# burritojustice/reporter

Hardware: AMD Instinct MI355X
Metric: GPS points matched/sec (whole node) at 1/2/4/8 MI355X; % segment-ID agreement vs meili (higher is better)
Workload: dtype f32

## Files before the change

reporter_amd/csrc/abi.cpp:

```cpp
#include <dlfcn.h>

#include <algorithm>
#include <atomic>
#include <chrono>
#include <cmath>
#include <condition_variable>
#include <cstdio>
#include <cstdlib>
#include <cstring>
#include <deque>
#include <fstream>
#include <exception>
#include <functional>
#include <memory>
#include <mutex>
#include <new>
#include <sstream>
#include <thread>

#include "engine.h"
#include "javastr.h"
#include "json.h"
#include "pyrepr.h"
#include "report.h"
// ... 1735 lines not shown
  E->nbins = dev_counts ? nbins : 0;
  E->bin_kph = bin_kph;
  return OTM_OK;
}

int otm_hist_bind(otm_engine* E, void* dev_counts, int nbins, float bin_kph) {
  return otm_hist_bind_ex(E, dev_counts, nbins, bin_kph, nullptr);
}

int otm_graph_info(const otm_engine* E, int64_t* n_nodes, int64_t* n_edges, int64_t* n_segments) {
  if (!E) return fail(OTM_EINVAL, "engine is NULL");
  if (!E->members.empty()) E = E->members[0];
  if (n_nodes) *n_nodes = E->host.h.n_nodes;
  if (n_edges) *n_edges = E->host.h.n_edges;
  if (n_segments) *n_segments = E->host.h.n_segments;
  return OTM_OK;
}

int otm_index_info(const otm_engine* E, float* rmax, int64_t* entries, int32_t* incomplete_rows, float* build_ms) {
  if (!E) return fail(OTM_EINVAL, "engine is NULL");
  if (!E->members.empty()) E = E->members[0];
  if (rmax) *rmax = E->idx.rmax;
  if (entries) *entries = E->index_entries;
  if (incomplete_rows) *incomplete_rows = E->index_incomplete_rows;
  if (build_ms) *build_ms = E->index_build_ms;
  return OTM_OK;
}

int otm_index_tables(const otm_engine* E, int64_t* slots, int64_t* bytes, int32_t* load_pct) {
  if (!E) return fail(OTM_EINVAL, "engine is NULL");
  if (!E->members.empty()) E = E->members[0];
  const int64_t n = E->index_slots + E->index_near_slots;
  if (slots) *slots = n;
  if (bytes) *bytes = n * otm::IDX_SLOT_BYTES;
  if (load_pct) *load_pct = E->idx.rmax > 0.0f ? E->idx.load_pct : 0;
  return OTM_OK;
}

int otm_index_levels(const otm_engine* E, float* radii, int64_t* entries, int cap) {
  if (!E) return fail(OTM_EINVAL, "engine is NULL");
  if (!E->members.empty()) E = E->members[0];
  int n = 0;
  for (int l = 0; l < otm::NEAR_LEVELS; ++l) {
    if (!(E->idxn[l].rmax > 0.0f)) continue;
    if (n < cap) {
      if (radii) radii[n] = E->idxn[l].rmax;
      if (entries) entries[n] = E->index_near_level_entries[l];
    }
    ++n;
  }
  return n;
}

int otm_grid_info(const otm_engine* E, double* cell_deg, int32_t* rows, int32_t* cols, int64_t* entries,
                  int32_t* mult) {
  if (!E) return fail(OTM_EINVAL, "engine is NULL");
  if (!E->members.empty()) E = E->members[0];
  if (cell_deg) *cell_deg = E->g.cell;
  if (rows) *rows = E->grid_rows;
  if (cols) *cols = E->grid_cols;
  if (entries) *entries = E->grid_entries;
  if (mult) *mult = E->grid_mult;
  return OTM_OK;
}

int otm_set_counting(otm_engine* E, int on) {
  if (!E) return fail(OTM_EINVAL, "engine is NULL");
// ... 173 lines not shown
```

reporter_amd/csrc/engine.cpp:

```cpp
#include "engine.h"

#include <algorithm>
#include <chrono>
#include <cmath>
#include <cstdlib>

#include <cstring>

namespace otm {

#define HIPCHK(x)                                                              \
  do {                                                                         \
    hipError_t e_ = (x);                                                       \
    if (e_ != hipSuccess) {                                                    \
      *err = std::string(#x) + ": " + hipGetErrorString(e_);                   \
      return OTM_EDEVICE;                                                      \
    }                                                                          \
  } while (0)

static int ensure(otm_engine::Buf& b, size_t bytes, std::string* err);
static int ensure_pinned(otm_engine::Buf& b, size_t bytes, std::string* err) {
  if (bytes == 0) bytes = 16;
  if (b.cap >= bytes) return OTM_OK;
  if (b.p) (void)hipHostFree(b.p);
// ... 297 lines not shown

int create_stream(int slot, hipStream_t* s, bool own_queue) {
  (void)slot;
  if (own_queue) {
    int dev = 0, ncu = 0;
    if (hipGetDevice(&dev) == hipSuccess &&
        hipDeviceGetAttribute(&ncu, hipDeviceAttributeMultiprocessorCount, dev) == hipSuccess && ncu > 0) {
      std::vector<uint32_t> mask((size_t)(ncu + 31) / 32, 0u);
      for (int c = 0; c < ncu; ++c) mask[(size_t)c / 32] |= 1u << (c % 32);
      if (hipExtStreamCreateWithCUMask(s, (uint32_t)mask.size(), mask.data()) == hipSuccess) return 0;
    }
  }
  return hipStreamCreateWithFlags(s, hipStreamNonBlocking) != hipSuccess;
}

int engine_clone(const otm_engine* P, otm_engine* C, std::string* err, bool own_queue) {
  C->parent = P;
  C->device = P->device;
  HIPCHK(hipSetDevice(C->device));
  const int slot = ++const_cast<otm_engine*>(P)->n_clones;
  if (create_stream(slot, &C->stream, own_queue)) {
    *err = "stream creation failed";
    return OTM_EDEVICE;
  }
  C->host.h = P->host.h;
  C->g = P->g;
  C->idx = P->idx;
  for (int l = 0; l < NEAR_LEVELS; ++l) C->idxn[l] = P->idxn[l];
  for (int l = 0; l < NEAR_LEVELS; ++l) C->index_near_level_entries[l] = P->index_near_level_entries[l];
  C->index_rmax = P->index_rmax;
  C->index_entries = P->index_entries;
  C->index_slots = P->index_slots;
  C->index_near_slots = P->index_near_slots;
  C->index_incomplete_rows = P->index_incomplete_rows;
  C->index_build_ms = P->index_build_ms;
  C->small_points = P->small_points;
  C->trans_lanes = P->trans_lanes;
  C->mc = P->mc;
  C->rc = P->rc;
  C->dp = P->dp;
  C->drc = P->drc;
  HIPCHK(hipMalloc((void**)&C->ctr, sizeof(DevCounters)));
  HIPCHK(hipMalloc((void**)&C->ctr_save, sizeof(DevCounters)));
  HIPCHK(hipMemset(C->ctr, 0, sizeof(DevCounters)));
  for (auto& e : C->kev) HIPCHK(hipEventCreate(&e));
  (void)err;
  return OTM_OK;
}

static float auto_index_radius(const otm_engine* E) {
  constexpr double INDEX_ROW_NODES = 140.0;
  const auto& h = E->host.h;
  const double lat_mid = 0.5 * (h.bbox[0] + h.bbox[2]) * 3.14159265358979323846 / 180.0;
  const double h_m = (h.bbox[2] - h.bbox[0]) * 111195.0;
  const double w_m = (h.bbox[3] - h.bbox[1]) * 111195.0 * std::cos(lat_mid);
  const double area = std::max(h_m * w_m, 1.0);
  const double rho = std::max((double)h.n_nodes, 1.0) / area;
  double r = std::sqrt(INDEX_ROW_NODES / (2.0 * rho));
  r = std::min(r, (double)E->dp.factor * (double)E->dp.breakage);
  return (float)(std::ceil(r / 50.0) * 50.0);
}

namespace {
struct IndexBuilt {
  DevIndex X{};
  int64_t entries = 0, slots = 0;
  int32_t incomplete = 0;
};
int build_index_at(otm_engine* E, float* r, bool shrink, size_t budget, IndexBuilt& out, std::string* err) {
  out = IndexBuilt{};
  const int32_t N = E->g.n_edges + E->g.n_nodes;
  hipStream_t s = E->stream;
  int32_t* row_cnt = nullptr;
  int64_t* row_off = nullptr;
  IdxRow* rows = nullptr;
  HIPCHK(hipMalloc(&row_cnt, ((size_t)N + 1) * 4));
  HIPCHK(hipMalloc(&row_off, ((size_t)N + 1) * 8));
  HIPCHK(hipMalloc(&rows, ((size_t)N + 1) * sizeof(IdxRow)));
  size_t tmpb = scan_tmp_bytes(N) + 256;
  void* tmp = nullptr;
  HIPCHK(hipMalloc(&tmp, tmpb));
  int64_t total = 0;
  int pct = index_load_fast();
  auto size_rows = [&](int load) -> int {
    launch_row_sizes(row_cnt, row_off, N, load, s);
    scan_i64(row_off, N, tmp, tmpb, s);
    launch_row_pack(row_cnt, row_off, rows, N, s);
    HIPCHK(hipMemcpyAsync(&total, row_off + N, 8, hipMemcpyDeviceToHost, s));
    HIPCHK(hipStreamSynchronize(s));
    return OTM_OK;
  };
  for (int attempt = 0;; ++attempt) {
    launch_index_build(E->g, E->dp.turn_units, index_cost_bound(*r), row_cnt, nullptr, nullptr, false, s);
    if (size_rows(pct)) return OTM_EDEVICE;
    if (pct != index_load_dense() && ((double)total + 1.0) * IDX_SLOT_BYTES > (double)budget) {
      pct = index_load_dense();
      if (size_rows(pct)) return OTM_EDEVICE;
    }
    const double need = ((double)total + 1.0) * IDX_SLOT_BYTES;
    if (need <= (double)budget) break;
    const float rr = (float)(std::floor(*r * std::sqrt((double)budget / need) * 0.9 / 50.0) * 50.0);
    if (!shrink || attempt == 4 || rr < 100.0f) {
      (void)hipFree(tmp);
      (void)hipFree(rows);
      (void)hipFree(row_off);
      (void)hipFree(row_cnt);
      *r = 0.0f;
      return OTM_OK;
    }
    *r = rr;
  }
  (void)hipFree(tmp);
  E->graph_allocs.push_back(row_cnt);
  E->graph_allocs.push_back(row_off);
  E->graph_allocs.push_back(rows);
  void* slot = nullptr;
  HIPCHK(hipMalloc(&slot, ((size_t)total + 1) * IDX_SLOT_BYTES));
  E->graph_allocs.push_back(slot);
  HIPCHK(hipMemsetAsync(slot, 0xFF, ((size_t)total + 1) * IDX_SLOT_BYTES, s));
  launch_index_build(E->g, E->dp.turn_units, index_cost_bound(*r), row_cnt, rows, (uint4*)slot, true, s);
  HIPCHK(hipGetLastError());
  std::vector<int32_t> cnt((size_t)N);
  HIPCHK(hipMemcpyAsync(cnt.data(), row_cnt, (size_t)N * 4, hipMemcpyDeviceToHost, s));
  HIPCHK(hipStreamSynchronize(s));
  for (int32_t c : cnt) {
    out.incomplete += c < 0;
    out.entries += c > 0 ? c : 0;
  }
  out.slots = total;
  out.X.rmax = *r;
  out.X.cmax = index_cost_bound(*r);
  out.X.row = rows;
  out.X.slot = (const uint4*)slot;
  out.X.load_pct = pct;
  return OTM_OK;
}

size_t index_budget() {
  if (const char* bm = std::getenv("OTM_INDEX_BUDGET_MB")) return (size_t)std::strtoull(bm, nullptr, 0) << 20;
  size_t fr = 0, tot = 0;
  if (hipMemGetInfo(&fr, &tot) != hipSuccess) return 0;
  return fr / 2;
}
}

int build_index(otm_engine* E, std::string* err) {
  E->idx = DevIndex{};
  for (auto& x : E->idxn) x = DevIndex{};
  E->idx.rmax = 0.0f;
  if (E->index_rmax < 0.0f) E->index_rmax = auto_index_radius(E);
  E->index_rmax = std::min(E->index_rmax, INDEX_RMAX_CAP);
  if (!(E->index_rmax > 0.0f)) return OTM_OK;
  hipStream_t s = E->stream;
  hipEvent_t a, z;
  HIPCHK(hipEventCreate(&a));
  HIPCHK(hipEventCreate(&z));
  HIPCHK(hipEventRecord(a, s));
  IndexBuilt full;
  int rc = build_index_at(E, &E->index_rmax, true, index_budget(), full, err);
  if (rc != OTM_OK) return rc;
  E->idx = full.X;
  E->index_entries = full.entries;
  E->index_slots = full.slots;
  E->index_incomplete_rows = full.incomplete;
  std::vector<float> radii;
  if (E->index_near_set) {
    radii = E->index_near_m;
  } else if ((double)full.slots * IDX_SLOT_BYTES >= OTM_INDEX_NEAR_MIN_GB * 1e9) {
    for (float f : std::initializer_list<float> OTM_INDEX_NEAR_FRACS) radii.push_back(E->index_rmax * f);
  }
  for (float& r : radii) r = (float)(std::floor(r / 50.0) * 50.0);
  std::sort(radii.begin(), radii.end());
  radii.erase(std::unique(radii.begin(), radii.end()), radii.end());
  int nl = 0;
  for (float rn : radii) {
    if (nl == NEAR_LEVELS || !(E->idx.rmax > 0.0f) || rn < 100.0f || rn >= E->idx.rmax) continue;
    IndexBuilt near;
    rc = build_index_at(E, &rn, false, index_budget(), near, err);
    if (rc != OTM_OK) return rc;
    if (rn > 0.0f) {
      E->index_near_level_entries[nl] = near.entries;
      E->index_near_slots += near.slots;
      E->idxn[nl++] = near.X;
    }
  }
  HIPCHK(hipEventRecord(z, s));
  HIPCHK(hipEventSynchronize(z));
  HIPCHK(hipEventElapsedTime(&E->index_build_ms, a, z));
  (void)hipEventDestroy(a);
  (void)hipEventDestroy(z);
  return OTM_OK;
}

void engine_free(otm_engine* E) {
  if (E->device >= 0) (void)hipSetDevice(E->device);
  for (void* p : E->graph_allocs) (void)hipFree(p);
  E->graph_allocs.clear();
  otm_engine::Buf* bufs[] = {
      &E->in_off,        &E->in_lat,       &E->in_lon,         &E->in_time,        &E->in_acc,     &E->in_blob,
      &E->pt_trace,
      &E->is_col,        &E->prevc,        &E->nextc,        &E->gc,             &E->ncand,          &E->cand_eo,      &E->cand_em,
      &E->cand_xeo,      &E->cand_xem,
      &E->probe,         &E->col_prev,     &E->kq_prev,        &E->vmeta,  &E->colrec, &E->colrec_pos,        &E->trans_off,      &E->trans,          &E->bp,         &E->state,      &E->chosen,
      &E->chain_start,   &E->route_dist,   &E->ipos,   &E->path_off,       &E->path_len,       &E->path_pool,  &E->trace_err,
      &E->overflow_list0, &E->overflow_list2, &E->counters_i32, &E->scan_tmp, &E->snap,   &E->big_key,
      &E->big_lab,       &E->big_inq,      &E->big_fr,         &E->big_ins,        &E->big_prev,
      &E->huge_key,      &E->huge_lab,     &E->huge_inq,       &E->huge_fr,        &E->huge_ins,         &E->huge_prev,
      &E->cbig_key,      &E->cbig_val,     &E->cbig_skey,
      &E->overflow_list3, &E->o_traces,       &E->o_seg_cnt,  &E->o_way_cnt,
      &E->o_segments,    &E->o_seg_gidx,   &E->o_way_ids,      &E->o_reports,  &E->o_rep_cnt,  &E->seg_ub,
      &E->f_seg_off,     &E->f_way_off,    &E->f_rep_off,      &E->f_segs,     &E->f_ways,     &E->f_reps,
      &E->f_traces,
      &E->abort_flag,    &E->rs_blob,      &E->ord_tile,      &E->ord_cnt,      &E->ord_cursor,     &E->ord_grp,    &E->ord_item,
      &E->d_req,         &E->req_cnt,      &E->req_ok,     &E->req_lat,    &E->req_lon,    &E->req_time,   &E->req_acc,
      &E->resp_hdr,      &E->resp_seg,     &E->resp_rep,       &E->resp_hlen,      &E->resp_slen,  &E->resp_rlen,
// ... 981 lines not shown
```

reporter_amd/csrc/engine.h:

```cpp
#pragma once
#include <atomic>
#include <hip/hip_runtime.h>

#include <condition_variable>
#include <deque>
#include <memory>
#include <mutex>
#include <string>
#include <thread>
#include <vector>

#include "kernels.h"
#include "otm_internal.h"
#include "otmatch.h"

struct ReqSlab {
  char* base = nullptr;
  size_t cap = 0;
  bool pinned = false;
};

namespace otm {
struct H2DOrder {
  std::mutex m;
// ... 5 lines not shown
};
}

struct otm_engine {
  const otm_engine* parent = nullptr;
  std::vector<otm_engine*> members;
  struct MemberPool* member_pool = nullptr;
  std::vector<otm_trace_result> g_traces;
  std::vector<otm_segment> g_segs;
  std::vector<otm_report_rec> g_reps;
  std::vector<int64_t> g_ways;
  int device = 0;
  std::atomic<int> n_clones{0};
  hipStream_t stream = nullptr;
  hipEvent_t sync_ev = nullptr;
  bool spin_waits = false;
  otm::HostGraph host;
  otm::DevGraph g{};
  std::vector<void*> graph_allocs;
  float index_rmax = -1.0f;
  int64_t small_points = 0;
  int trans_lanes = 8;
  int grid_mult = 0;
  int32_t grid_rows = 0, grid_cols = 0;
  int64_t grid_entries = 0;
  otm::DevIndex idx{};
  otm::DevIndex idxn[otm::NEAR_LEVELS]{};
  std::vector<float> index_near_m;
  bool index_near_set = false;
  int64_t index_near_level_entries[otm::NEAR_LEVELS]{};
  int64_t index_entries = 0;
  int64_t index_slots = 0;
  int64_t index_near_slots = 0;
  int32_t index_incomplete_rows = 0;
  float index_build_ms = 0.0f;
  otm::MatchConfig mc;
  otm::ReportConfig rc;
  otm::DevParams dp{};
  otm::DevReportCfg drc{};
  std::mutex mu;

  struct Buf {
    void* p = nullptr;
    size_t cap = 0;
  };
  Buf in_off, in_lat, in_lon, in_time, in_acc, in_blob;
  Buf pt_trace, is_col, prevc, nextc, gc, ncand, cand_eo, cand_em, cand_xeo, cand_xem, probe, col_prev, kq_prev, vmeta, colrec, colrec_pos, trans_off, trans, bp, state, chosen,
      chain_start, route_dist, ipos, path_off, path_len, path_pool, trace_err, overflow_list0, overflow_list2,
      counters_i32, scan_tmp, snap;
  Buf big_key, big_lab, big_inq, big_fr, big_ins, big_prev;
  Buf huge_key, huge_lab, huge_inq, huge_fr, huge_ins, huge_prev, overflow_list3;
  int32_t huge_log2 = 0;
  int32_t huge_ready_log2 = 0;
  Buf cbig_key, cbig_val, cbig_skey;
  int32_t cand_log2 = 0;
  int32_t huge_final = 0, cand_final = 0;
  int32_t last_attempts = 0;
  int32_t last_resumes = 0;
  Buf ord_tile, ord_cnt, ord_cursor, ord_grp, ord_item;
  Buf abort_flag;
  Buf rs_blob;
  int64_t trans_cap = 0;
  bool caps_read = false, caps_pinned = false;
  Buf o_traces, o_seg_cnt, o_way_cnt, o_rep_cnt, seg_ub, o_segments, o_seg_gidx, o_way_ids, o_reports;
  Buf f_seg_off, f_way_off, f_rep_off, f_segs, f_ways, f_reps, f_traces;
  otm::DevCounters* ctr = nullptr;
// ... 87 lines not shown
```

reporter_amd/csrc/kernels.h:

```cpp
#pragma once
#include <hip/hip_runtime.h>

#include <cstdint>

#include "otmatch.h"

namespace otm {

constexpr int KMAX = 32;
constexpr int KIN = 8;
static_assert(KIN == 4 || KIN == 8, "inline blocks of 4 or 8 slots (whole 16-B emission pieces)");
constexpr int KX = KMAX - KIN;
constexpr int MAX_HITS = 256;
constexpr int SEARCH_LIMIT = 98304;
constexpr int LDS_TABLE_CAP = 256;
constexpr int LDS_TABLE_LIMIT = 192;
constexpr int BIG_TABLE_LOG2 = 17;
constexpr int BIG_TABLE_CAP = 1 << BIG_TABLE_LOG2;
#ifndef OTM_BIG_SLOTS
#define OTM_BIG_SLOTS 512
#endif
constexpr int BIG_SLOTS = OTM_BIG_SLOTS;
constexpr int HUGE_SLOTS = 8;
constexpr int CAND_BIG_SLOTS = 64;
// ... 15 lines not shown
  const uint32_t* cell_off;
  const uint32_t* cell_ent;
  const float4* ent_geo;
  const uint16_t *e_head_out, *e_head_in;
  const uint32_t* e_len64;
  const uint4* e_rec;
  const int2* e_fl;
  const int64_t* way_tab;
  int32_t n_nodes, n_edges, n_segments, grid_rows, grid_cols;
  double lat0, lon0, cell;
  float bb_lat0, bb_lon0, bb_inv_h, bb_inv_w;
};

#ifndef OTM_ORDER_BITS
#define OTM_ORDER_BITS 6
#endif
constexpr int ORDER_BITS = OTM_ORDER_BITS;
constexpr int ORDER_SIDE = 1 << ORDER_BITS;
constexpr int ORDER_TILES = ORDER_SIDE * ORDER_SIDE;
constexpr int ORDER_GROUPS = 8;
struct DevOrder {
  int32_t* item;
  int32_t* grp;
  uint16_t* tile;
  int32_t* tile_cnt;
  int32_t* cursor;
};

struct IdxRow {
  int64_t off;
  int32_t cnt;
  uint32_t cap;
};
struct DevIndex {
  float rmax;
  uint32_t cmax;
  const IdxRow* row;
  const uint4* slot;
  int load_pct;
};
constexpr int IDX_SLOT_BYTES = 16;
constexpr float INDEX_RMAX_CAP = 200000.0f;
constexpr uint32_t NODE_KEY = 0x80000000u;
constexpr uint32_t NONE_PRED = 0xFFFFFFFFu;
constexpr int NEAR_LEVELS = 3;
#ifndef OTM_INDEX_NEAR_FRACS
#define OTM_INDEX_NEAR_FRACS {0.45f}
#endif
#ifndef OTM_INDEX_NEAR_MIN_GB
#define OTM_INDEX_NEAR_MIN_GB 16.0
#endif
constexpr int INDEX_BUILD_LOG2 = 11;
constexpr int INDEX_BUILD_CAP = 1 << INDEX_BUILD_LOG2;
constexpr int INDEX_BUILD_LIMIT = 1536;
__host__ __device__ inline uint32_t index_cost_bound(float B) { return (uint32_t)floor((double)B * 64.0); }

constexpr int ORDER_CAND = 1, ORDER_TRANS = 2, ORDER_ROUTE = 4;
constexpr int TURN_TABLE = 181;
constexpr uint32_t TURN_UNITS_MAX = 0xFFFFFFu;
constexpr uint32_t NO_TURNS = 0xFFFFFFFFu;
struct DevParams {
  float sigma_z, beta, factor, breakage, interp, search_radius, max_search_radius, gps_accuracy;
  const uint32_t* turn_units;
  int max_candidates;
  int order_mask;
  int cand_wave_all;
};

struct DevReportCfg {
  int n_report, n_transition;
// ... 138 lines not shown
void launch_transitions(const DevGraph& g, const DevBatch& b, const DevParams& p, DevWork& w, hipStream_t s,
                        const Marks& mk, int sub, int from = RESUME_ALL);
void launch_viterbi(const DevBatch& b, DevWork& w, hipStream_t s, const Marks& mk);
void launch_route(const DevGraph& g, const DevBatch& b, const DevParams& p, DevWork& w, hipStream_t s,
                  const Marks& mk, int from = RESUME_ALL);
void launch_segments(const DevGraph& g, const DevBatch& b, DevWork& w, DevOut& o, bool write, hipStream_t s,
                     const Marks& mk);
void launch_report(const DevBatch& b, const DevReportCfg& rc, DevWork& w, DevOut& o, hipStream_t s, const Marks& mk);
void launch_order(const DevBatch& b, DevWork& w, hipStream_t s, const Marks& mk);
void launch_seg_bound(const DevGraph& g, const DevBatch& b, const DevParams& p, DevWork& w, int64_t* tb, hipStream_t s,
                      const Marks& mk);
void launch_compact(int32_t n_traces, const DevOut& o, const int32_t* seg_off, const int32_t* way_off,
                    const int32_t* rep_off, void* segs_out, int64_t* ways_out, void* reps_out, void* traces_out,
                    hipStream_t s);
void launch_index_build(const DevGraph& g, const uint32_t* turn_units, uint32_t cmax, int32_t* row_cnt,
                        const IdxRow* rows, uint4* slot, bool write, hipStream_t s);
int index_load_fast();
int index_load_dense();
void launch_row_sizes(const int32_t* row_cnt, int64_t* row_sizes, int32_t n, int pct, hipStream_t s);
struct BatchStatus {
  int32_t abort, grow;
  int64_t ttotal;
  int32_t cnt[3];
  int32_t route_huge;
};
void launch_batch_init(int32_t* counters, int32_t* abort, hipStream_t s);
void launch_expand_compact(const int64_t* trace_off, const int64_t* tbase, const int32_t* dt, const int16_t* acc16,
                           double* time, float* acc, int32_t n_traces, hipStream_t s);
void launch_snap(int32_t* counters, int32_t* snap, bool reset, hipStream_t s);
bool fold_bookkeeping();
void launch_status(const int32_t* abort, const int64_t* ttotal, const int32_t* counters, BatchStatus* out,
                   hipStream_t s);
void launch_row_pack(const int32_t* row_cnt, const int64_t* row_off, IdxRow* rows, int32_t n, hipStream_t s);
size_t req_sparse_slots(int32_t n, size_t bytes);
void launch_req_read(const unsigned char* blob, const int64_t* off, int32_t r0, int32_t r1, int32_t n, int64_t* cnt,
                     uint8_t* ok, const DevBatch& sparse, hipStream_t s);
void launch_req_compact(const int64_t* off, int32_t n, const int64_t* pre, const uint8_t* ok, const DevBatch& sparse,
                        const DevBatch& out, int64_t* trace_off, hipStream_t s);
constexpr int RESP_HDR_SLOT = 512;
constexpr int RESP_SEG_SLOT = 320;
constexpr int RESP_REP_SLOT = 192;
struct RespIn {
  int32_t nt, ns, nr;
  const otm_trace_result* traces;
  const otm_segment* segs;
  const int64_t* ways;
  const otm_report_rec* reps;
};
struct RespWork {
  char *hdr, *seg, *rep;
  int32_t *hlen, *slen, *rlen;
  int64_t* blen;
  uint8_t* host;
};
size_t resp_seg_scratch(int32_t ns, int32_t nw);
void launch_resp_items(const RespIn& in, const RespWork& w, hipStream_t s);
void launch_resp_len(const RespIn& in, const RespWork& w, hipStream_t s);
void launch_resp_copy(const RespIn& in, const RespWork& w, const int64_t* boff, char* blob, hipStream_t s);
void scan_i64(int64_t* d, int64_t n, void* tmp, size_t tmp_bytes, hipStream_t s);
constexpr int FETCH_SCAN_MAX = 1 << 16;
void launch_fetch_scan(int32_t n, const int32_t* c0, const int32_t* c1, const int32_t* c2, int32_t* o0, int32_t* o1,
                       int32_t* o2, hipStream_t s);
void scan_i32(int32_t* d, int64_t n, void* tmp, size_t tmp_bytes, hipStream_t s);
size_t scan_tmp_bytes(int64_t n);

}
// ... 1 lines not shown
```

reporter_amd/csrc/kernels.hip:

```cpp
#include <hip/hip_runtime.h>

#include <algorithm>
#include <cstdlib>
#include <type_traits>

#include <hipcub/hipcub.hpp>

#include "kernels.h"
#include "otmatch.h"

namespace otm {

namespace {

#define MPD_F 111319.4954833f
constexpr uint32_t EMPTY = 0xFFFFFFFFu;
constexpr unsigned long long LAB_NONE = ~0ull;
constexpr int TB = 64;
__device__ __forceinline__ void wave_sync() {
  __builtin_amdgcn_wave_barrier();
  asm volatile("" ::: "memory");
}

__device__ __forceinline__ float cos_deg(float deg) {
// ... 402 lines not shown
  int64_t i0, i1, stride;
  bool ordered;
};
__device__ __forceinline__ ItemRange item_range(const DevWork& w, const DevBatch& b, bool ordered, int per_block) {
  ItemRange r;
  r.ordered = ordered;
  const int tid = per_block > 1 ? (int)threadIdx.x : 0;
  if (ordered) {
    const int grp = blockIdx.x % ORDER_GROUPS;
    r.i0 = w.ord.grp[grp] + (int64_t)(blockIdx.x / ORDER_GROUPS) * per_block + tid;
    r.i1 = w.ord.grp[grp + 1];
    r.stride = (int64_t)(gridDim.x / ORDER_GROUPS) * per_block;
  } else {
    r.i0 = (int64_t)blockIdx.x * per_block + tid;
    r.i1 = b.n_points;
    r.stride = (int64_t)gridDim.x * per_block;
  }
  return r;
}

constexpr int HCAP = 512;
constexpr uint32_t NODE_ENT = 0x80000000u;
#ifndef OTM_CAND_LANE_CAP
#define OTM_CAND_LANE_CAP 8
#endif
constexpr int CAND_LANE_CAP = OTM_CAND_LANE_CAP;
#ifndef OTM_CAND_TB
#define OTM_CAND_TB 256
#endif
#ifndef OTM_CAND_WAVES
#define OTM_CAND_WAVES 8
#endif
constexpr int CAND_TB = OTM_CAND_TB;
#ifndef OTM_CAND_INFL
#define OTM_CAND_INFL 2
#endif
constexpr int CAND_INFL = OTM_CAND_INFL;
#ifndef OTM_SNAP_B
#define OTM_SNAP_B 2
#endif
constexpr int SNAP_B = OTM_SNAP_B;
#ifndef OTM_TRANS_BATCH
#define OTM_TRANS_BATCH 1
#endif

__device__ __forceinline__ void wave_cadd(unsigned long long* c, unsigned long long v) {
  for (int o = 32; o > 0; o >>= 1) v += __shfl_xor(v, o, 64);
  if ((threadIdx.x & 63) == 0 && v) atomicAdd(c, v);
}

template <bool CTR>
__global__ __launch_bounds__(CAND_TB, OTM_CAND_WAVES) void k_cand_lane(DevGraph g, DevBatch b, DevParams P, DevWork w) {
  __shared__ uint32_t sE[CAND_LANE_CAP * CAND_TB];
  __shared__ float sQ[CAND_LANE_CAP * CAND_TB];
  uint32_t* E = sE + threadIdx.x;
  float* Q = sQ + threadIdx.x;
  constexpr int S = CAND_TB;
  unsigned long long c_cells = 0, c_ent = 0, c_cand = 0;
  const ItemRange R = item_range(w, b, (P.order_mask & ORDER_CAND) != 0, CAND_TB);
  for (int64_t it = R.i0; it < R.i1; it += R.stride) {
    const int64_t p = R.ordered ? (int64_t)w.ord.item[it] : it;
    if (!R.ordered && !w.is_col[p]) continue;
    if (P.cand_wave_all) {
      const int slot = atomicAdd(&w.counters_i32[5], 1);
      w.overflow_list0[slot] = (int32_t)p;
      continue;
    }
    const float4 pr = w.probe[p];
    const float lat = pr.x, lon = pr.y;
    const float r = probe_radius(P, pr.z);
    const float r2 = r * r;
    const float ls = MPD_F * cos_deg(lat);
    const float dlat = r / MPD_F;
    const float dlon = r / ls;
    const double la_lo = ((double)lat - (double)dlat - g.lat0) / g.cell;
    const double la_hi = ((double)lat + (double)dlat - g.lat0) / g.cell;
    const double lo_lo = ((double)lon - (double)dlon - g.lon0) / g.cell;
    const double lo_hi = ((double)lon + (double)dlon - g.lon0) / g.cell;
    const double R = g.grid_rows, Cn = g.grid_cols;
    int r0 = 0, r1 = -1, c0 = 0, c1 = -1;
    if (!(la_hi < 0.0 || lo_hi < 0.0 || la_lo >= R || lo_lo >= Cn)) {
      r0 = la_lo < 0.0 ? 0 : (int)floor(la_lo);
      r1 = la_hi >= R ? (int)R - 1 : (int)floor(la_hi);
      c0 = lo_lo < 0.0 ? 0 : (int)floor(lo_lo);
      c1 = lo_hi >= Cn ? (int)Cn - 1 : (int)floor(lo_hi);
    }
    int n = 0;
    bool spill = false;
    const unsigned long long cells = (unsigned long long)(r1 - r0 + 1) * (unsigned long long)(c1 - c0 + 1);
// ... 24 lines not shown
            if (spill || !(sqd <= r2)) continue;
            const uint32_t ent = en[u];
            const uint32_t e = ent >> 4;
            uint32_t ev[CAND_LANE_CAP];
#pragma unroll
            for (int m = 0; m < CAND_LANE_CAP; ++m) ev[m] = E[m * S];
            int f = -1;
#pragma unroll
            for (int m = 0; m < CAND_LANE_CAP; ++m) f = (m < n && (ev[m] >> 4) == e) ? m : f;
            if (f < 0) {
              if (n == CAND_LANE_CAP) {
                spill = true;
                continue;
              }
              E[n * S] = ent;
              Q[n * S] = sqd;
              ++n;
            } else {
              const float qf = Q[f * S];
              if (sqd < qf || (sqd == qf && (ent & 15u) < (E[f * S] & 15u))) {
                Q[f * S] = sqd;
                E[f * S] = ent;
              }
            }
          }
        }
      }
    }
    if (spill) {
      const int slot = atomicAdd(&w.counters_i32[5], 1);
      w.overflow_list0[slot] = (int32_t)p;
      continue;
    }
    for (int m0 = 0; m0 < n; m0 += SNAP_B) {
      uint32_t em[SNAP_B];
      ProjIn pin[SNAP_B];
#pragma unroll
      for (int u = 0; u < SNAP_B; ++u) {
        em[u] = m0 + u < n ? E[(m0 + u) * S] : 0u;
        if (m0 + u < n) pin[u] = proj_load(g, (int32_t)(em[u] >> 4), (int32_t)(em[u] & 15u));
      }
      int32_t vx[SNAP_B];
      bool node0[SNAP_B], at_end[SNAP_B];
#pragma unroll
      for (int u = 0; u < SNAP_B; ++u) {
        vx[u] = 0;
        node0[u] = at_end[u] = false;
        if (m0 + u < n) {
          float sqd, off;
          proj_calc(pin[u], lat, lon, ls, sqd, off, at_end[u]);
          node0[u] = off == 0.0f;
          const int32_t e = (int32_t)(em[u] >> 4);
          if (node0[u] || at_end[u]) vx[u] = node0[u] ? g.e_from[e] : g.e_to[e];
        }
      }
#pragma unroll
      for (int u = 0; u < SNAP_B; ++u) {
        if (node0[u] || at_end[u]) {
          const int32_t o0 = g.out_off[vx[u]], o1 = g.out_off[vx[u] + 1];
          if (node0[u] || o1 > o0) E[(m0 + u) * S] = NODE_ENT | ((uint32_t)o0 << 4);
        }
      }
    }
    for (int m = 0; m < n; ++m) {
      const uint32_t key = E[m * S];
      if (!(key & NODE_ENT)) continue;
      int f = -1;
      for (int t = 0; t < m; ++t)
        if (E[t * S] == key) f = t;
      if (f >= 0) {
        const float qm = Q[m * S];
        if (qm < Q[f * S]) Q[f * S] = qm;
        --n;
        E[m * S] = E[n * S];
        Q[m * S] = Q[n * S];
        --m;
      }
    }
    const int K = n < P.max_candidates ? n : P.max_candidates;
    const float ds = (2.0f * P.sigma_z) * P.sigma_z;
    for (int j = 0; j < K; ++j) {
      int m = j;
      float qm = Q[j * S];
      uint32_t em = E[j * S];
      for (int t = j + 1; t < n; ++t) {
        const float qt = Q[t * S];
        const uint32_t et = E[t * S];
        const uint32_t xt = (et & ~NODE_ENT) >> 4, xm = (em & ~NODE_ENT) >> 4;
        if (qt < qm || (qt == qm && (xt < xm || (xt == xm && et > em)))) {
          m = t;
          qm = qt;
          em = et;
        }
      }
      if (m != j) {
        Q[m * S] = Q[j * S];
        E[m * S] = E[j * S];
        Q[j * S] = qm;
        E[j * S] = em;
      }
    }
    int4* eo4 = (int4*)(w.cand_eo + p * KIN);
    float4* em4 = (float4*)(w.cand_em + p * KIN);
    float emv[4];
#pragma unroll
    for (int j = 0; j < (CAND_LANE_CAP > KIN ? CAND_LANE_CAP : KIN); j += 2) {
      if (j >= KIN && j >= K) break;
      int32_t e2[2];
      float o2[2];
#pragma unroll
      for (int u = 0; u < 2; ++u) {
        const int jj = j + u;
        e2[u] = -1;
        o2[u] = 0.0f;
        float emj = INFINITY;
        if (jj < K) {
          const uint32_t en = E[jj * S];
          const int32_t e = (int32_t)((en & ~NODE_ENT) >> 4);
          float sqd = Q[jj * S], off = 0.0f;
          if (!(en & NODE_ENT)) project(g, e, (int32_t)(en & 15u), lat, lon, ls, sqd, off);
          e2[u] = e;
          o2[u] = off;
          emj = sqd / ds;
        }
        emv[(j + u) & 3] = emj;
      }
      if (j < KIN) {
        eo4[j >> 1] = make_int4(e2[0], __float_as_int(o2[0]), e2[1], __float_as_int(o2[1]));
        if ((j & 3) == 2) em4[j >> 2] = make_float4(emv[0], emv[1], emv[2], emv[3]);
      } else {
#pragma unroll
        for (int u = 0; u < 2; ++u)
          if (j + u < K) {
            w.cand_xeo[p * KX + (j + u - KIN)] = make_int2(e2[u], __float_as_int(o2[u]));
            w.cand_xem[p * KX + (j + u - KIN)] = emv[(j + u) & 3];
          }
      }
    }

    w.ncand[p] = K;
    if (CTR) {
      c_cells += cells;
      c_ent += ents;
      c_cand += (unsigned long long)K;
    }
  }
  if (CTR) {
    wave_cadd(&w.ctr->cells_visited, c_cells);
    wave_cadd(&w.ctr->cell_entries_scanned, c_ent);
    wave_cadd(&w.ctr->candidates, c_cand);
  }
}

// ... 588 lines not shown
      uint32_t h = idx_slot0(idx_hash(k), R);
      while (atomicCAS(&slot[R.off + h].x, EMPTY, k) != EMPTY) h = idx_next(h, R);
      slot[R.off + h].y = (uint32_t)(lab >> 32) & IDX_LOW24;
      slot[R.off + h].z = fbits(d);
      slot[R.off + h].w = units & IDX_LOW24;
    }
    __syncthreads();
    for (int i = lane; i < INDEX_BUILD_CAP; i += TB) {
      const uint32_t k = lkey[i];
      if (k == EMPTY) continue;
      const uint32_t pk = (uint32_t)(llab[i] & 0xFFFFFFFFull);
      uint4 sk_v, tmp;
      const int64_t sk = idx_find(slot, R, k, sk_v);
      const int64_t sp = pk == NONE_PRED ? -1 : idx_find(slot, R, pk, tmp);
      const uint32_t ps = sp < 0 ? IDX_NO_PRED : (uint32_t)(sp - R.off);
      slot[sk].y = (sk_v.y & IDX_LOW24) | (ps & 0xFFu) << 24;
      slot[sk].w = (sk_v.w & IDX_LOW24) | (ps >> 8) << 24;
    }
    __syncthreads();
  }
}

__global__ void k_row_sizes(const int32_t* row_cnt, int64_t* sizes, int32_t n, int pct) {
  const int32_t u = blockIdx.x * blockDim.x + threadIdx.x;
  if (u < n) sizes[u] = idx_row_cap(row_cnt[u], pct);
  if (u == n) sizes[n] = 0;
}

__global__ void k_row_pack(const int32_t* row_cnt, const int64_t* row_off, IdxRow* rows, int32_t n) {
  const int32_t u = blockIdx.x * blockDim.x + threadIdx.x;
  if (u >= n) return;
  const int64_t cap = row_off[u + 1] - row_off[u];
  rows[u] = IdxRow{row_off[u], row_cnt[u], (uint32_t)cap};
}

#ifndef OTM_TRANS_KC8
#define OTM_TRANS_KC8 8
#endif
#ifndef OTM_TRANS_WAVES
#define OTM_TRANS_WAVES 8
#endif
template <int S, bool LIST>
__global__ __launch_bounds__(TB, OTM_TRANS_WAVES) void k_trans_sub(DevGraph g, DevBatch b, DevParams P, DevWork w) {
  if (*w.abort || trans_over_cap(b, w)) return;
  static_assert(S == 8 || S == 16, "8 lanes per column (two passes) or 16 (one pass / the wide pass)");
  constexpr int NS = TB / S;
  constexpr int KC = S >= 16 ? 16 : OTM_TRANS_KC8;
  constexpr bool WIDE = KC < 16;
  __shared__ int4 tg[NS][KC];
  __shared__ int4 sr[NS][KC];
  __shared__ IdxRow rq[NS][KC];
#ifndef OTM_TRANS_SWZ
#define OTM_TRANS_SWZ 1
#endif
  const int lane = threadIdx.x, sg = lane / S, sl = lane % S;
  const unsigned long long smask = ((1ull << S) - 1ull) << (sg * S);
  const int swz = !OTM_TRANS_SWZ ? 0 : (S == 8 ? ((sg >> 1) & 1) * 4 : (sg & 1) * 8);
  const DevIndex& X = w.idx;
  unsigned long long c_search = 0, c_settled = 0, c_relaxed = 0, c_trans = 0;
  const bool ordered = !LIST && (P.order_mask & ORDER_TRANS) != 0;
  int64_t base, end, stride;
  if (LIST) {
    base = (int64_t)blockIdx.x * NS;
    end = w.counters_i32[6];
    stride = (int64_t)gridDim.x * NS;
  } else if (ordered) {
// ... 4 lines not shown
  } else {
    base = (int64_t)blockIdx.x * NS;
    end = b.n_points;
    stride = (int64_t)gridDim.x * NS;
  }
  for (; base < end; base += stride) {
    const int64_t it = base + sg;
    bool act = it < end;
    int64_t p = 0;
    int32_t q = -1;
    int Kp = 0, Kq = 0;
    float gcv = 0.0f;
    int64_t toff = 0;
    if (act && ordered && w.colrec) {
      const int4 A = w.colrec[it];
      p = A.x;
      toff = w.trans_off[p];
      q = A.y;
      Kq = A.z & 255;
      Kp = A.z >> 8;
      gcv = __int_as_float(A.w);
    } else if (act) {
      p = LIST ? (int64_t)w.overflow_list2[it] : (ordered ? (int64_t)w.ord.item[it] : it);
      q = w.col_prev[p];
      Kq = w.kq_prev[p];
      Kp = w.ncand[p];
      gcv = w.gc[p];
      toff = w.trans_off[p];
    }
    act = act && q >= 0;
    const float bound = P.factor * gcv;
    const uint32_t cq = index_cost_bound(bound);
    const bool idx_ok = X.rmax > 0.0f && cq <= X.cmax;
    const IdxRow* xrow = X.row;
    const uint4* xslot = X.slot;
#pragma unroll
    for (int l = NEAR_LEVELS - 1; l >= 0; --l) {
      if (w.idxn[l].rmax > 0.0f && cq <= w.idxn[l].cmax) {
        xrow = w.idxn[l].row;
        xslot = w.idxn[l].slot;
      }
    }
    const bool wide = WIDE && act && idx_ok && (Kp > KC || Kq > KC);
    if (wide && sl == 0) w.overflow_list2[atomicAdd(&w.counters_i32[6], 1)] = (int32_t)p;
    act = act && !wide;
    bool bad = act && (!idx_ok || Kp > KC || Kq > KC);
    for (int k = sl; k < KC; k += S) {
      if (act && k < Kp) {
        const int2 c = crec(w, p, k);
        const int32_t e = c.x;
        const float o = __int_as_float(c.y);
        const uint32_t key = dst_key(g, e, o);
        tg[sg][k ^ swz] = make_int4(e, __float_as_int(o), (int)key, (int)idx_hash(key));
      }
      if (act && k < Kq) {
        const int2 c = crec(w, q, k);
        const int32_t e = c.x;
        const float o = __int_as_float(c.y);
        const int2 fl = g.e_fl[e];
        const float start = cand_node(o) ? 0.0f : __int_as_float(fl.y) - o;
        sr[sg][k ^ swz] = make_int4(e, __float_as_int(o), __float_as_int(start), w.ctr ? (int)src_head(g, e, o) : 0);
        if (idx_ok) {
          const IdxRow R = xrow[cand_node(o) ? (int64_t)g.n_edges + fl.x : (int64_t)e];
          rq[sg][k ^ swz] = R;
          bad = bad || R.cnt < 0;
        }
      }
    }
    const bool spill = (__ballot(bad) & smask) != 0ull;
    if (spill && act && sl == 0) {
      const int slot = atomicAdd(&w.counters_i32[4], 1);
      w.overflow_list0[slot] = (int32_t)p;
    }
    act = act && !spill;
    wave_sync();
    if (act) {
      float* Tm = w.trans + toff;
      unsigned long long ntr = 0;
      constexpr int NB = OTM_TRANS_BATCH;
      const int npair = Kq * Kp;
      for (int idx0 = sl; idx0 < npair; idx0 += S * NB) {
        uint4 s0[NB], s1[NB];
        uint32_t h0[NB];
#pragma unroll
        for (int u = 0; u < NB; ++u) {
          const int idx = idx0 + u * S;
          s0[u] = make_uint4(EMPTY, 0u, 0u, 0u);
          s1[u] = s0[u];
          h0[u] = 0u;
          if (idx < npair) {
            const int i = idx / Kp, j = idx - (idx / Kp) * Kp;
            const int4 T = tg[sg][j ^ swz], Sx = sr[sg][i ^ swz];
            const IdxRow R = rq[sg][i ^ swz];
            const bool same = same_edge_step(Sx.x, __int_as_float(Sx.y), T.x, __int_as_float(T.y));
            if (!same && R.cnt > 0) {
              h0[u] = idx_slot0((uint32_t)T.w, R);
              s0[u] = xslot[R.off + h0[u]];
              s1[u] = xslot[R.off + h0[u] + 1];
            }
// ... 101 lines not shown
      p = A.x;
      q = A.y;
      gcv = __int_as_float(A.w);
    } else {
      p = R.ordered ? (int64_t)w.ord.item[it] : it;
    }
    if (!R.ordered && !w.is_col[p]) continue;
    w.route_dist[p] = 0.0f;
    w.path_len[p] = 0;
    w.path_off[p] = 0;
    const int2 cq0 = w.chosen[q >= 0 ? q : p];
    if (w.state[p] < 0 || w.chain_start[p]) continue;
    if (!rec) {
      q = w.col_prev[p];
      gcv = w.gc[p];
    }
    const int2 ci = rec ? cq0 : w.chosen[q], cj = w.chosen[p];
    const int32_t ei = ci.x, ej = cj.x;
    const float oi = __int_as_float(ci.y), oj = __int_as_float(cj.y);
    if (same_edge_step(ei, oi, ej, oj)) {
      w.route_dist[p] = same_edge_dist(oi, oj);
      continue;
    }
    const float bound = P.factor * gcv;
    const uint32_t cq = index_cost_bound(bound);
    IdxRow Rw{};
    int64_t sv = -1;
    uint4 lab{};
    int lvl = -1;
#pragma unroll
    for (int l = NEAR_LEVELS - 1; l >= 0; --l)
      if (w.idxn[l].rmax > 0.0f && cq <= w.idxn[l].cmax) lvl = l;
    const DevIndex& Xc = lvl >= 0 ? w.idxn[lvl] : X;
    const int2 fli = g.e_fl[ei];
    if (X.rmax > 0.0f && cq <= X.cmax) {
      Rw = Xc.row[cand_node(oi) ? (int64_t)g.n_edges + fli.x : (int64_t)ei];
      sv = idx_find(Xc.slot, Rw, dst_key(g, ej, oj), lab);
    }
    if (sv < 0 || idx_slot_cost(lab) > cq) {
      const int slot = atomicAdd(&w.counters_i32[4], 1);
      w.overflow_list0[slot] = (int32_t)p;
      continue;
    }
    int len = 0;
    for (int32_t ps = idx_slot_pred(lab); ps >= 0 && len <= Rw.cnt; ps = idx_slot_pred(Xc.slot[Rw.off + ps])) ++len;
    const int off = len ? atomicAdd(&w.counters_i32[1], len) : 0;
    if (off + len > w.pool_cap) {
      w.counters_i32[2] = 1;
      *w.abort = 1;
      w.path_len[p] = -1;
    } else {
      int k = len;
      for (int32_t ps = idx_slot_pred(lab); ps >= 0 && k > 0;) {
        const uint4 sl = Xc.slot[Rw.off + ps];
        w.path_pool[off + (--k)] = (int32_t)sl.x;
        ps = idx_slot_pred(sl);
      }
      w.path_off[p] = off;
      w.path_len[p] = len;
    }
    const float start = cand_node(oi) ? 0.0f : __int_as_float(fli.y) - oi;
    const float sd = start + bitsf(lab.z);
    w.route_dist[p] = sd + oj;
    if (w.ctr) {
      unsigned long long st = 0, rl = 0;
      for (int64_t k = 0; k < (int64_t)Rw.cap; ++k) {
        const uint4 sl = Xc.slot[Rw.off + k];
        if (sl.x == EMPTY || (sl.x & NODE_KEY) || idx_slot_cost(sl) > cq) continue;
        ++st;
        if ((unsigned long long)idx_slot_cost(sl) + g.e_len64[sl.x] <= cq) {
          const int32_t v = g.e_to[sl.x];
          rl += (unsigned long long)(g.out_off[v + 1] - g.out_off[v]);
        }
      }
      ++c_search;
      c_settled += st;
      c_relaxed += rl;
      c_edges += (unsigned long long)len;
    }
  }
  if (w.ctr) {
    cadd(&w.ctr->route_searches, c_search);
    cadd(&w.ctr->route_nodes_settled, c_settled);
    cadd(&w.ctr->route_edges_relaxed, c_relaxed);
    cadd(&w.ctr->route_edges, c_edges);
  }
}

template <int TIER>
__device__ __forceinline__ Table tier_table(const DevWork& w, uint32_t* lkey, unsigned long long* llab, uint32_t* linq,
                                            uint32_t* lfr0, uint32_t* lfr1) {
  if (TIER == 1) {
    const size_t base = (size_t)blockIdx.x * BIG_TABLE_CAP;
    return Table{w.big_key + base, w.big_lab + base, w.big_inq + base, w.big_fr + 2 * base,
// ... 2129 lines not shown
  hipLaunchKernelGGL(k_compact, dim3(grid_for(n_traces, 1, WAVE_GRID_CAP)), dim3(TB), 0, s, n_traces, o, seg_off, way_off,
                     rep_off, (otm_segment*)segs_out, ways_out, (otm_report_rec*)reps_out,
                     (otm_trace_result*)traces_out);
}
void launch_report(const DevBatch& b, const DevReportCfg& rc, DevWork& w, DevOut& o, hipStream_t s,
                   const Marks& mk) {
  constexpr int tb = 16;
  if (OTM_REPORT_FORM == 1 || (OTM_REPORT_FORM == 2 && b.n_traces <= REPW_MAX_TRACES))
    TIMED(KN_REPORT, hipLaunchKernelGGL(k_report_wave, dim3(grid_for(b.n_traces, 1, WAVE_GRID_CAP)), dim3(TB), 0, s,
                                        b, rc, w, o, 0));
  else
    TIMED(KN_REPORT, hipLaunchKernelGGL(k_report, dim3(grid_for(b.n_traces, tb, 1 << 30)), dim3(tb), 0, s, b, rc, w,
                                        o, 0));
}
#undef TIMED

void launch_index_build(const DevGraph& g, const uint32_t* turn_units, uint32_t cmax, int32_t* row_cnt,
                        const IdxRow* rows, uint4* slot, bool write, hipStream_t s) {
  const int grid = grid_for((int64_t)g.n_edges + g.n_nodes, 1, 256 * 16);
  if (write)
    hipLaunchKernelGGL(k_index_build<true>, dim3(grid), dim3(TB), 0, s, g, turn_units, cmax, row_cnt, rows, slot);
  else
    hipLaunchKernelGGL(k_index_build<false>, dim3(grid), dim3(TB), 0, s, g, turn_units, cmax, row_cnt, rows, slot);
}
int index_load_fast() { return IDX_LOAD_FAST; }
int index_load_dense() { return IDX_LOAD_DENSE; }
void launch_row_sizes(const int32_t* row_cnt, int64_t* row_sizes, int32_t n, int pct, hipStream_t s) {
  hipLaunchKernelGGL(k_row_sizes, dim3(grid_for((int64_t)n + 1, 256, 1 << 30)), dim3(256), 0, s, row_cnt, row_sizes,
                     n, pct);
}
void launch_row_pack(const int32_t* row_cnt, const int64_t* row_off, IdxRow* rows, int32_t n, hipStream_t s) {
  hipLaunchKernelGGL(k_row_pack, dim3(grid_for((int64_t)n, 256, 1 << 30)), dim3(256), 0, s, row_cnt, row_off, rows, n);
}

size_t scan_tmp_bytes(int64_t n) {
  size_t a = 0, c = 0;
  (void)hipcub::DeviceScan::ExclusiveSum(nullptr, a, (int64_t*)nullptr, (int64_t*)nullptr, (int)(n + 1));
  (void)hipcub::DeviceScan::ExclusiveSum(nullptr, c, (int32_t*)nullptr, (int32_t*)nullptr, (int)(n + 1));
  return a > c ? a : c;
}
void scan_i64(int64_t* d, int64_t n, void* tmp, size_t tmp_bytes, hipStream_t s) {
  (void)hipcub::DeviceScan::ExclusiveSum(tmp, tmp_bytes, d, d, (int)(n + 1), s);
}
void scan_i32(int32_t* d, int64_t n, void* tmp, size_t tmp_bytes, hipStream_t s) {
  (void)hipcub::DeviceScan::ExclusiveSum(tmp, tmp_bytes, d, d, (int)(n + 1), s);
}

}
```

Baseline: 1.477 billion.

## Pack per-edge index rows into source records and keep projection offsets in registers

Adds a per-edge SrcRec array holding the edge's index row, its from-node's index row, from-node id and length. Transition and path kernels now fetch these with one contiguous record load instead of separate e_fl and row-table lookups. The candidate kernel also keeps projection offsets in registers with a 3-bit permutation tracker, so it no longer re-projects each kept candidate. The cost is extra device memory for the records, which is counted in the index budget and may shrink the index radius, plus more register pressure in the candidate kernel.

```diff
diff --git a/reporter_amd/csrc/abi.cpp b/reporter_amd/csrc/abi.cpp
--- a/reporter_amd/csrc/abi.cpp
+++ b/reporter_amd/csrc/abi.cpp
@@ -1791,7 +1791,7 @@
   if (!E->members.empty()) E = E->members[0];
   const int64_t n = E->index_slots + E->index_near_slots;
   if (slots) *slots = n;
-  if (bytes) *bytes = n * otm::IDX_SLOT_BYTES;
+  if (bytes) *bytes = n * otm::IDX_SLOT_BYTES + E->index_src_bytes;
   if (load_pct) *load_pct = E->idx.rmax > 0.0f ? E->idx.load_pct : 0;
   return OTM_OK;
 }
diff --git a/reporter_amd/csrc/engine.cpp b/reporter_amd/csrc/engine.cpp
--- a/reporter_amd/csrc/engine.cpp
+++ b/reporter_amd/csrc/engine.cpp
@@ -353,6 +353,7 @@
   C->index_entries = P->index_entries;
   C->index_slots = P->index_slots;
   C->index_near_slots = P->index_near_slots;
+  C->index_src_bytes = P->index_src_bytes;
   C->index_incomplete_rows = P->index_incomplete_rows;
   C->index_build_ms = P->index_build_ms;
   C->small_points = P->small_points;
@@ -385,7 +386,7 @@
 namespace {
 struct IndexBuilt {
   DevIndex X{};
-  int64_t entries = 0, slots = 0;
+  int64_t entries = 0, slots = 0, src_bytes = 0;
   int32_t incomplete = 0;
 };
 int build_index_at(otm_engine* E, float* r, bool shrink, size_t budget, IndexBuilt& out, std::string* err) {
@@ -403,6 +404,7 @@
   HIPCHK(hipMalloc(&tmp, tmpb));
   int64_t total = 0;
   int pct = index_load_fast();
+  const double src_bytes = (double)E->g.n_edges * sizeof(SrcRec);
   auto size_rows = [&](int load) -> int {
     launch_row_sizes(row_cnt, row_off, N, load, s);
     scan_i64(row_off, N, tmp, tmpb, s);
@@ -414,11 +416,11 @@
   for (int attempt = 0;; ++attempt) {
     launch_index_build(E->g, E->dp.turn_units, index_cost_bound(*r), row_cnt, nullptr, nullptr, false, s);
     if (size_rows(pct)) return OTM_EDEVICE;
-    if (pct != index_load_dense() && ((double)total + 1.0) * IDX_SLOT_BYTES > (double)budget) {
+    if (pct != index_load_dense() && ((double)total + 1.0) * IDX_SLOT_BYTES + src_bytes > (double)budget) {
       pct = index_load_dense();
       if (size_rows(pct)) return OTM_EDEVICE;
     }
-    const double need = ((double)total + 1.0) * IDX_SLOT_BYTES;
+    const double need = ((double)total + 1.0) * IDX_SLOT_BYTES + src_bytes;
     if (need <= (double)budget) break;
     const float rr = (float)(std::floor(*r * std::sqrt((double)budget / need) * 0.9 / 50.0) * 50.0);
     if (!shrink || attempt == 4 || rr < 100.0f) {
@@ -441,6 +443,11 @@
   HIPCHK(hipMemsetAsync(slot, 0xFF, ((size_t)total + 1) * IDX_SLOT_BYTES, s));
   launch_index_build(E->g, E->dp.turn_units, index_cost_bound(*r), row_cnt, rows, (uint4*)slot, true, s);
   HIPCHK(hipGetLastError());
+  SrcRec* src = nullptr;
+  HIPCHK(hipMalloc(&src, ((size_t)E->g.n_edges + 1) * sizeof(SrcRec)));
+  E->graph_allocs.push_back(src);
+  launch_src_pack(E->g, rows, src, s);
+  HIPCHK(hipGetLastError());
   std::vector<int32_t> cnt((size_t)N);
   HIPCHK(hipMemcpyAsync(cnt.data(), row_cnt, (size_t)N * 4, hipMemcpyDeviceToHost, s));
   HIPCHK(hipStreamSynchronize(s));
@@ -452,6 +459,8 @@
   out.X.rmax = *r;
   out.X.cmax = index_cost_bound(*r);
   out.X.row = rows;
+  out.X.src = src;
+  out.src_bytes = (int64_t)E->g.n_edges * (int64_t)sizeof(SrcRec);
   out.X.slot = (const uint4*)slot;
   out.X.load_pct = pct;
   return OTM_OK;
@@ -483,6 +492,7 @@
   E->idx = full.X;
   E->index_entries = full.entries;
   E->index_slots = full.slots;
+  E->index_src_bytes = full.src_bytes;
   E->index_incomplete_rows = full.incomplete;
   std::vector<float> radii;
   if (E->index_near_set) {
@@ -502,6 +512,7 @@
     if (rn > 0.0f) {
       E->index_near_level_entries[nl] = near.entries;
       E->index_near_slots += near.slots;
+      E->index_src_bytes += near.src_bytes;
       E->idxn[nl++] = near.X;
     }
   }
diff --git a/reporter_amd/csrc/engine.h b/reporter_amd/csrc/engine.h
--- a/reporter_amd/csrc/engine.h
+++ b/reporter_amd/csrc/engine.h
@@ -61,6 +61,7 @@
   int64_t index_entries = 0;
   int64_t index_slots = 0;
   int64_t index_near_slots = 0;
+  int64_t index_src_bytes = 0;
   int32_t index_incomplete_rows = 0;
   float index_build_ms = 0.0f;
   otm::MatchConfig mc;
diff --git a/reporter_amd/csrc/kernels.h b/reporter_amd/csrc/kernels.h
--- a/reporter_amd/csrc/kernels.h
+++ b/reporter_amd/csrc/kernels.h
@@ -71,10 +71,26 @@
   int32_t cnt;
   uint32_t cap;
 };
+#ifndef OTM_SRC_REC
+#define OTM_SRC_REC 1
+#endif
+#ifndef OTM_SRC_REC_BYTES
+#define OTM_SRC_REC_BYTES 48
+#endif
+struct alignas(16) SrcRec {
+  IdxRow edge;
+  IdxRow node;
+  int32_t from;
+  int32_t len;
+  int32_t pad[(OTM_SRC_REC_BYTES - 40) / 4];
+};
+static_assert(sizeof(SrcRec) == OTM_SRC_REC_BYTES && (OTM_SRC_REC_BYTES == 48 || OTM_SRC_REC_BYTES == 64),
+              "source records of 48 or 64 bytes");
 struct DevIndex {
   float rmax;
   uint32_t cmax;
   const IdxRow* row;
+  const SrcRec* src;
   const uint4* slot;
   int load_pct;
 };
@@ -279,6 +295,7 @@
 void launch_status(const int32_t* abort, const int64_t* ttotal, const int32_t* counters, BatchStatus* out,
                    hipStream_t s);
 void launch_row_pack(const int32_t* row_cnt, const int64_t* row_off, IdxRow* rows, int32_t n, hipStream_t s);
+void launch_src_pack(const DevGraph& g, const IdxRow* rows, SrcRec* src, hipStream_t s);
 size_t req_sparse_slots(int32_t n, size_t bytes);
 void launch_req_read(const unsigned char* blob, const int64_t* off, int32_t r0, int32_t r1, int32_t n, int64_t* cnt,
                      uint8_t* ok, const DevBatch& sparse, hipStream_t s);
diff --git a/reporter_amd/csrc/kernels.hip b/reporter_amd/csrc/kernels.hip
--- a/reporter_amd/csrc/kernels.hip
+++ b/reporter_amd/csrc/kernels.hip
@@ -458,6 +458,9 @@
 #define OTM_CAND_WAVES 8
 #endif
 constexpr int CAND_TB = OTM_CAND_TB;
+#ifndef OTM_CAND_OFF
+#define OTM_CAND_OFF 2
+#endif
 #ifndef OTM_CAND_INFL
 #define OTM_CAND_INFL 2
 #endif
@@ -481,6 +484,12 @@
   __shared__ float sQ[CAND_LANE_CAP * CAND_TB];
   uint32_t* E = sE + threadIdx.x;
   float* Q = sQ + threadIdx.x;
+#if OTM_CAND_OFF == 1
+  __shared__ float sO[CAND_LANE_CAP * CAND_TB];
+  float* O = sO + threadIdx.x;
+#elif OTM_CAND_OFF == 2
+  static_assert(CAND_LANE_CAP <= 8 && CAND_LANE_CAP % SNAP_B == 0, "3-bit slots; whole snap steps");
+#endif
   constexpr int S = CAND_TB;
   unsigned long long c_cells = 0, c_ent = 0, c_cand = 0;
   const ItemRange R = item_range(w, b, (P.order_mask & ORDER_CAND) != 0, CAND_TB);
@@ -571,7 +580,17 @@
       w.overflow_list0[slot] = (int32_t)p;
       continue;
     }
+#if OTM_CAND_OFF == 2
+    float offr[CAND_LANE_CAP];
+    uint32_t perm = 076543210u;
+#pragma unroll
+    for (int m0 = 0; m0 < CAND_LANE_CAP; m0 += SNAP_B) {
+#pragma unroll
+      for (int u = 0; u < SNAP_B; ++u) offr[m0 + u] = 0.0f;
+      if (m0 >= n) continue;
+#else
     for (int m0 = 0; m0 < n; m0 += SNAP_B) {
+#endif
       uint32_t em[SNAP_B];
       ProjIn pin[SNAP_B];
 #pragma unroll
@@ -581,13 +600,16 @@
       }
       int32_t vx[SNAP_B];
       bool node0[SNAP_B], at_end[SNAP_B];
+      float offv[SNAP_B];
 #pragma unroll
       for (int u = 0; u < SNAP_B; ++u) {
         vx[u] = 0;
         node0[u] = at_end[u] = false;
+        offv[u] = 0.0f;
         if (m0 + u < n) {
           float sqd, off;
           proj_calc(pin[u], lat, lon, ls, sqd, off, at_end[u]);
+          offv[u] = off;
           node0[u] = off == 0.0f;
           const int32_t e = (int32_t)(em[u] >> 4);
           if (node0[u] || at_end[u]) vx[u] = node0[u] ? g.e_from[e] : g.e_to[e];
@@ -597,8 +619,16 @@
       for (int u = 0; u < SNAP_B; ++u) {
         if (node0[u] || at_end[u]) {
           const int32_t o0 = g.out_off[vx[u]], o1 = g.out_off[vx[u] + 1];
-          if (node0[u] || o1 > o0) E[(m0 + u) * S] = NODE_ENT | ((uint32_t)o0 << 4);
-        }
+          if (node0[u] || o1 > o0) {
+            E[(m0 + u) * S] = NODE_ENT | ((uint32_t)o0 << 4);
+            offv[u] = 0.0f;
+          }
+        }
+#if OTM_CAND_OFF == 1
+        if (m0 + u < n) O[(m0 + u) * S] = offv[u];
+#elif OTM_CAND_OFF == 2
+        offr[m0 + u] = offv[u];
+#endif
       }
     }
     for (int m = 0; m < n; ++m) {
@@ -613,6 +643,11 @@
         --n;
         E[m * S] = E[n * S];
         Q[m * S] = Q[n * S];
+#if OTM_CAND_OFF == 1
+        O[m * S] = O[n * S];
+#elif OTM_CAND_OFF == 2
+        perm = (perm & ~(7u << (3 * m))) | ((perm >> (3 * n)) & 7u) << (3 * m);
+#endif
         --m;
       }
     }
@@ -637,6 +672,14 @@
         E[m * S] = E[j * S];
         Q[j * S] = qm;
         E[j * S] = em;
+#if OTM_CAND_OFF == 1
+        const float om = O[m * S];
+        O[m * S] = O[j * S];
+        O[j * S] = om;
+#elif OTM_CAND_OFF == 2
+        const uint32_t x = ((perm >> (3 * m)) ^ (perm >> (3 * j))) & 7u;
+        perm ^= x << (3 * m) | x << (3 * j);
+#endif
       }
     }
     int4* eo4 = (int4*)(w.cand_eo + p * KIN);
@@ -656,8 +699,18 @@
         if (jj < K) {
           const uint32_t en = E[jj * S];
           const int32_t e = (int32_t)((en & ~NODE_ENT) >> 4);
+#if OTM_CAND_OFF == 0
           float sqd = Q[jj * S], off = 0.0f;
           if (!(en & NODE_ENT)) project(g, e, (int32_t)(en & 15u), lat, lon, ls, sqd, off);
+#elif OTM_CAND_OFF == 1
+          const float sqd = Q[jj * S], off = O[jj * S];
+#else
+          const float sqd = Q[jj * S];
+          const uint32_t sl = (perm >> (3 * jj)) & 7u;
+          float off = offr[0];
+#pragma unroll
+          for (int t = 1; t < CAND_LANE_CAP; ++t) off = sl == (uint32_t)t ? offr[t] : off;
+#endif
           e2[u] = e;
           o2[u] = off;
           emj = sqd / ds;
@@ -1312,6 +1365,26 @@
   if (u >= n) return;
   const int64_t cap = row_off[u + 1] - row_off[u];
   rows[u] = IdxRow{row_off[u], row_cnt[u], (uint32_t)cap};
+}
+
+__global__ void k_src_pack(DevGraph g, const IdxRow* rows, SrcRec* src) {
+  const int32_t e = blockIdx.x * blockDim.x + threadIdx.x;
+  if (e >= g.n_edges) return;
+  const int2 fl = g.e_fl[e];
+  SrcRec r{};
+  r.edge = rows[e];
+  r.node = rows[(int64_t)g.n_edges + fl.x];
+  r.from = fl.x;
+  r.len = fl.y;
+  src[e] = r;
+}
+__device__ __forceinline__ IdxRow src_row(const SrcRec* src, int32_t e, bool node) {
+  const uint4 v = ((const uint4*)(src + e))[node ? 1 : 0];
+  IdxRow R;
+  R.off = (int64_t)((unsigned long long)v.x | (unsigned long long)v.y << 32);
+  R.cnt = (int32_t)v.z;
+  R.cap = v.w;
+  return R;
 }
 
 #ifndef OTM_TRANS_KC8
@@ -1382,12 +1455,20 @@
     const float bound = P.factor * gcv;
     const uint32_t cq = index_cost_bound(bound);
     const bool idx_ok = X.rmax > 0.0f && cq <= X.cmax;
+#if OTM_SRC_REC
+    const SrcRec* xsrc = X.src;
+#else
     const IdxRow* xrow = X.row;
+#endif
     const uint4* xslot = X.slot;
 #pragma unroll
     for (int l = NEAR_LEVELS - 1; l >= 0; --l) {
       if (w.idxn[l].rmax > 0.0f && cq <= w.idxn[l].cmax) {
+#if OTM_SRC_REC
+        xsrc = w.idxn[l].src;
+#else
         xrow = w.idxn[l].row;
+#endif
         xslot = w.idxn[l].slot;
       }
     }
@@ -1407,6 +1488,22 @@
         const int2 c = crec(w, q, k);
         const int32_t e = c.x;
         const float o = __int_as_float(c.y);
+#if OTM_SRC_REC
+        IdxRow R{};
+        int32_t lenb;
+        if (idx_ok) {
+          R = src_row(xsrc, e, cand_node(o));
+          lenb = xsrc[e].len;
+        } else {
+          lenb = g.e_fl[e].y;
+        }
+        const float start = cand_node(o) ? 0.0f : __int_as_float(lenb) - o;
+        sr[sg][k ^ swz] = make_int4(e, __float_as_int(o), __float_as_int(start), w.ctr ? (int)src_head(g, e, o) : 0);
+        if (idx_ok) {
+          rq[sg][k ^ swz] = R;
+          bad = bad || R.cnt < 0;
+        }
+#else
         const int2 fl = g.e_fl[e];
         const float start = cand_node(o) ? 0.0f : __int_as_float(fl.y) - o;
         sr[sg][k ^ swz] = make_int4(e, __float_as_int(o), __float_as_int(start), w.ctr ? (int)src_head(g, e, o) : 0);
@@ -1415,6 +1512,7 @@
           rq[sg][k ^ swz] = R;
           bad = bad || R.cnt < 0;
         }
+#endif
       }
     }
     const bool spill = (__ballot(bad) & smask) != 0ull;
@@ -1582,11 +1680,21 @@
     for (int l = NEAR_LEVELS - 1; l >= 0; --l)
       if (w.idxn[l].rmax > 0.0f && cq <= w.idxn[l].cmax) lvl = l;
     const DevIndex& Xc = lvl >= 0 ? w.idxn[lvl] : X;
+#if OTM_SRC_REC
+    int32_t leni = 0;
+    if (X.rmax > 0.0f && cq <= X.cmax) {
+      Rw = src_row(Xc.src, ei, cand_node(oi));
+      leni = Xc.src[ei].len;
+      sv = idx_find(Xc.slot, Rw, dst_key(g, ej, oj), lab);
+    }
+#else
     const int2 fli = g.e_fl[ei];
+    const int32_t leni = fli.y;
     if (X.rmax > 0.0f && cq <= X.cmax) {
       Rw = Xc.row[cand_node(oi) ? (int64_t)g.n_edges + fli.x : (int64_t)ei];
       sv = idx_find(Xc.slot, Rw, dst_key(g, ej, oj), lab);
     }
+#endif
     if (sv < 0 || idx_slot_cost(lab) > cq) {
       const int slot = atomicAdd(&w.counters_i32[4], 1);
       w.overflow_list0[slot] = (int32_t)p;
@@ -1609,7 +1717,7 @@
       w.path_off[p] = off;
       w.path_len[p] = len;
     }
-    const float start = cand_node(oi) ? 0.0f : __int_as_float(fli.y) - oi;
+    const float start = cand_node(oi) ? 0.0f : __int_as_float(leni) - oi;
     const float sd = start + bitsf(lab.z);
     w.route_dist[p] = sd + oj;
     if (w.ctr) {
@@ -3805,6 +3913,10 @@
 void launch_row_pack(const int32_t* row_cnt, const int64_t* row_off, IdxRow* rows, int32_t n, hipStream_t s) {
   hipLaunchKernelGGL(k_row_pack, dim3(grid_for((int64_t)n, 256, 1 << 30)), dim3(256), 0, s, row_cnt, row_off, rows, n);
 }
+void launch_src_pack(const DevGraph& g, const IdxRow* rows, SrcRec* src, hipStream_t s) {
+  if (g.n_edges <= 0) return;
+  hipLaunchKernelGGL(k_src_pack, dim3(grid_for((int64_t)g.n_edges, 256, 1 << 30)), dim3(256), 0, s, g, rows, src);
+}
 
 size_t scan_tmp_bytes(int64_t n) {
   size_t a = 0, c = 0;
```

Measured after the change: 1.501 billion (median of 6 runs). 1.7% higher.
